# timsainb/noisereduce

Hardware: AMD Instinct MI355X
Metric: Msamples/s reduce_noise (48 kHz mono, n_fft=1024) (higher is better)
Workload: dtype f32

## Files before the change

noisereduce_amd/csrc/fastpath.hpp:

```cpp
#pragma once
#include "kernels.hpp"
#include "thresh.hpp"

namespace sg {

template <int NTHR, int COUNT, typename SLOW>
__device__ __forceinline__ void stage_t2_plain(float* s_t2, const double* __restrict__ T2, int need, double scale, int tid,
                                               SLOW slow) {
  if (need == 0) {
    constexpr int K = (COUNT + NTHR - 1) / NTHR;
    double t[K];
#pragma unroll
    for (int k = 0; k < K; ++k) t[k] = T2[min(tid + k * NTHR, COUNT - 1)];
#pragma unroll
    for (int k = 0; k < K; ++k) {
      const int i = tid + k * NTHR;
      if ((k + 1) * NTHR <= COUNT || i < COUNT) s_t2[i] = t2_to_f32(t[k], scale);
    }
  } else {
    for (int i = tid; i < COUNT; i += NTHR) s_t2[i] = t2_to_f32(slow(i), scale);
  }
}

template <typename ARGS>
__device__ __forceinline__ const ARGS* late_args() {
  const __attribute__((address_space(4))) char* kp = (const __attribute__((address_space(4))) char*)__builtin_amdgcn_kernarg_segment_ptr();
  asm volatile("" : "+s"(kp));
  return reinterpret_cast<const ARGS*>((const char*)kp);
}

namespace fast {

constexpr int FN = 512;
constexpr int FPITCH = FN + 16;
constexpr int WAVE_CX = 4 * FPITCH;
constexpr int FSK = 528;

typedef cx<float> cf;

template <int NTHR, int WIN4>
__device__ __forceinline__ void stage_tables(cf* tw512, const cf* __restrict__ tw_src, float* swin,
                                             const float* __restrict__ win_src, int tid) {
  constexpr bool WIN = WIN4 > 0;
  constexpr int K = (FN + NTHR - 1) / NTHR, KW = WIN ? (WIN4 + NTHR - 1) / NTHR : 1;
  cf t[K];
  float4 w[KW];
#pragma unroll
  for (int k = 0; k < K; ++k) {
    const int i = min(tid + k * NTHR, FN - 1);
    t[k] = tw_src[(i >> 4) * (i & 15)];
  }
  if constexpr (WIN) {
#pragma unroll
    for (int k = 0; k < KW; ++k) w[k] = reinterpret_cast<const float4*>(win_src)[min(tid + k * NTHR, WIN4 - 1)];
  }
#pragma unroll
  for (int k = 0; k < K; ++k) {
    const int i = tid + k * NTHR;
    if ((k + 1) * NTHR <= FN || i < FN) tw512[i] = t[k];
  }
  if constexpr (WIN) {
#pragma unroll
    for (int k = 0; k < KW; ++k) {
      const int i = tid + k * NTHR;
      if ((k + 1) * NTHR <= WIN4 || i < WIN4) reinterpret_cast<float4*>(swin)[i] = w[k];
    }
  }
}
template <int NTHR, int SPAN, int XPITCH, int ROW = 256, bool MX = false>
__device__ __forceinline__ unsigned stage_span_vec(float* xs, const float* __restrict__ sp, int tid) {
  static_assert(SPAN % 4 == 0, "16-byte loads");
  constexpr int N4 = SPAN / 4, NQ = (N4 + NTHR - 1) / NTHR;
  float4 q[NQ];
  unsigned mi = 0u;
#pragma unroll
  for (int k = 0; k < NQ; ++k) q[k] = reinterpret_cast<const float4*>(sp)[min(tid + k * NTHR, N4 - 1)];
#pragma unroll
  for (int k = 0; k < NQ; ++k) {
    const int e = 4 * (tid + k * NTHR);
    if ((k + 1) * NTHR <= N4 || e < SPAN) *reinterpret_cast<float4*>(&xs[(e / ROW) * XPITCH + (e % ROW)]) = q[k];
    if constexpr (MX) {
      auto ab = [](float x) -> unsigned { return __float_as_uint(x) & 0x7fffffffu; };
      mi = max(max(mi, max(ab(q[k].x), ab(q[k].y))), max(ab(q[k].z), ab(q[k].w)));
    }
  }
  return mi;
}

template <int NTHR, int SPAN, int XPITCH, int ROW = 256>
__device__ __forceinline__ void stage_span_vec_i16(float* xs, const int16_t* __restrict__ sp, int tid) {
  static_assert(SPAN % 4 == 0, "8-byte loads");
  constexpr int N4 = SPAN / 4, NQ = (N4 + NTHR - 1) / NTHR;
  uint2 q[NQ];
#pragma unroll
  for (int k = 0; k < NQ; ++k) q[k] = reinterpret_cast<const uint2*>(sp)[min(tid + k * NTHR, N4 - 1)];
#pragma unroll
  for (int k = 0; k < NQ; ++k) {
    const int e = 4 * (tid + k * NTHR);
    const float4 f = {(float)(short)(q[k].x & 0xffffu), (float)((int)q[k].x >> 16), (float)(short)(q[k].y & 0xffffu),
                      (float)((int)q[k].y >> 16)};
    if ((k + 1) * NTHR <= N4 || e < SPAN) *reinterpret_cast<float4*>(&xs[(e / ROW) * XPITCH + (e % ROW)]) = f;
  }
}

__device__ constexpr float C32[9] = {1.0f,
                                     0.98078528040323044913f,
                                     0.92387953251128675613f,
                                     0.83146961230254523708f,
                                     0.70710678118654752440f,
                                     0.55557023301960222474f,
                                     0.38268343236508977173f,
                                     0.19509032201612826785f,
                                     0.0f};

template <int R>
__device__ __forceinline__ constexpr float twc(int k) {
  int j = k * (32 / R);
  return j <= 8 ? C32[j] : -C32[16 - j];
}
template <int R>
__device__ __forceinline__ constexpr float tws(int k) {
  int j = k * (32 / R);
  return j <= 8 ? C32[8 - j] : C32[j - 8];
}

#ifndef SG_PK_FFT
#define SG_PK_FFT 0
#endif
typedef float pf2 __attribute__((ext_vector_type(2)));
__device__ __forceinline__ pf2 pk_of(cf a) { return pf2{a.x, a.y}; }
__device__ __forceinline__ cf pk_to(pf2 a) { return cf{a.x, a.y}; }
__device__ __forceinline__ pf2 pk_add(pf2 a, pf2 b) {
  pf2 d;
  asm("v_pk_add_f32 %0, %1, %2" : "=v"(d) : "v"(a), "v"(b));
  return d;
}
__device__ __forceinline__ pf2 pk_sub(pf2 a, pf2 b) {
  pf2 d;
  asm("v_pk_add_f32 %0, %1, %2 neg_lo:[0,1] neg_hi:[0,1]" : "=v"(d) : "v"(a), "v"(b));
  return d;
}
__device__ __forceinline__ pf2 pk_mul(pf2 a, pf2 b) {
  pf2 d;
  asm("v_pk_mul_f32 %0, %1, %2" : "=v"(d) : "v"(a), "v"(b));
  return d;
}
__device__ __forceinline__ pf2 pk_add_mi(pf2 a, pf2 b) {
  pf2 d;
  asm("v_pk_add_f32 %0, %1, %2 op_sel:[0,1] op_sel_hi:[1,0] neg_hi:[0,1]" : "=v"(d) : "v"(a), "v"(b));
  return d;
}
__device__ __forceinline__ pf2 pk_add_pi(pf2 a, pf2 b) {
  pf2 d;
  asm("v_pk_add_f32 %0, %1, %2 op_sel:[0,1] op_sel_hi:[1,0] neg_lo:[0,1]" : "=v"(d) : "v"(a), "v"(b));
  return d;
// ... 809 lines not shown
        float4 f4 = *reinterpret_cast<const float4*>(&fr[wh * WAVE_CX_H * 2 + lh * HPITCH + s4]);
        acc.x += f4.x; acc.y += f4.y; acc.z += f4.z; acc.w += f4.w;
      }
    } else {
#pragma unroll
      for (int q = 0; q < 4; ++q) {
        const int i = jj - q;
        const int64_t ti = tf_tile + i;
        if (i >= 0 && i < NF && ti >= 0 && ti < G.T) {
          const int off = ((i >> 2) * WAVE_CX + frame_base(i & 3)) * 2 + 256 * q + s4;
          float4 f4 = *reinterpret_cast<const float4*>(&fr[off]);
          acc.x += f4.x; acc.y += f4.y; acc.z += f4.z; acc.w += f4.w;
        }
      }
    }
    if (inkernel && jj >= NF) {
      unsigned long long* dst = A.part2 + (((size_t)u * A.n_tiles + bx) * 3 + (jj - NF)) * 256 + s4;
      const op_v4u ga = {__float_as_uint(acc.x), A.epoch, __float_as_uint(acc.y), A.epoch};
      const op_v4u gb = {__float_as_uint(acc.z), A.epoch, __float_as_uint(acc.w), A.epoch};
      op_st16_sc1(dst, ga);
      op_st16_sc1(dst + 2, gb);
      continue;
    }
    if (inkernel && jj < 3) {
      const unsigned long long* src = A.part2 + (((size_t)u * A.n_tiles + bx - 1) * 3 + jj) * 256 + s4;
      op_v4u ga, gb;
      for (int spin = 0;; ++spin) {
        asm volatile("global_load_dwordx4 %0, %2, off sc1\n\tglobal_load_dwordx4 %1, %2, off offset:16 sc1\n\ts_waitcnt vmcnt(0)"
                     : "=&v"(ga), "=&v"(gb) : "v"(src) : "memory");
        const unsigned e = A.epoch;
        if (!LOSE && ga[1] == e && ga[3] == e && gb[1] == e && gb[3] == e) break;
        if (LOSE || spin >= OP_SPIN_MAX) {
          atomicOr_system(A.err, 4u);
          ga[0] = ga[2] = gb[0] = gb[2] = 0x7fc00000u;
          break;
        }
        __builtin_amdgcn_s_sleep(1);
      }
      acc.x = __uint_as_float(ga[0]) + acc.x;
      acc.y = __uint_as_float(ga[2]) + acc.y;
      acc.z = __uint_as_float(gb[0]) + acc.z;
      acc.w = __uint_as_float(gb[2]) + acc.w;
    } else if (jj < 3 || jj >= NF) {
      const int slot = jj < 3 ? jj : 3 + (jj - NF);
      float* dst = A.part + (((u * A.n_tiles + bx) * 6 + slot) * 256 + s4);
      *reinterpret_cast<float4*>(dst) = acc;
      continue;
    }
    if (!A.normalize) {
    } else if (all_valid) {
      acc.x *= n4.x; acc.y *= n4.y; acc.z *= n4.z; acc.w *= n4.w;
    } else {
      float4 nrm = make_float4(0.f, 0.f, 0.f, 0.f);
#pragma unroll
      for (int q = 0; q < 4; ++q) {
        const int64_t ti = h - q;
        if (ti >= 0 && ti < G.T) {
          float4 w4 = *reinterpret_cast<const float4*>(&A.wsq[256 * q + s4]);
          nrm.x += w4.x; nrm.y += w4.y; nrm.z += w4.z; nrm.w += w4.w;
        }
      }
      acc.x /= (nrm.x > 1e-10f ? nrm.x : 1.f);
      acc.y /= (nrm.y > 1e-10f ? nrm.y : 1.f);
      acc.z /= (nrm.z > 1e-10f ? nrm.z : 1.f);
      acc.w /= (nrm.w > 1e-10f ? nrm.w : 1.f);
    }
    {
      const int64_t pb = h * 256 - G.padL;
      const int64_t gi0 = chunk * A.om.g_step + (pb - A.om.p0);
      if (A.om.dtype == 0 && pb >= A.om.p0 && pb + 256 <= A.om.p1 && pb + 256 <= G.Lout && gi0 >= A.om.g_lo &&
          gi0 + 256 <= A.om.g_hi && !(SG_ABLATE & 4)) {
        float* dst = (float*)A.om.out + (row * A.om.stride + gi0 - A.om.g0 + s4);
        if ((reinterpret_cast<uintptr_t>(dst) & 15) == 0) {
          *reinterpret_cast<float4*>(dst) = acc;
          continue;
        }
      }
    }
    const float vals[4] = {acc.x, acc.y, acc.z, acc.w};
#pragma unroll
    for (int e = 0; e < 4; ++e) {
      const int64_t p = h * 256 + s4 + e - G.padL;
      if (p < A.om.p0 || p >= A.om.p1) continue;
      const int64_t gi = chunk * A.om.g_step + (p - A.om.p0);
      if (gi < A.om.g_lo || gi >= A.om.g_hi) continue;
      if ((SG_ABLATE & 4) && vals[e] != 12345.678f) continue;
      store_sample(A.om.out, A.om.dtype, row * A.om.stride + gi - A.om.g0, p < G.Lout ? vals[e] : 0.f);
    }
  }
}

template <int NF>
__global__ __launch_bounds__(256) void k_ola_seam(ApplyArgs A) {
  const Geom& G = A.g;
  const int64_t u = blockIdx.y;
  const int64_t b = blockIdx.x;
  const int64_t row = (A.view.unit0 + u) / A.view.n_chunks;
  const int64_t chunk = A.view.c0 + (A.view.unit0 + u) % A.view.n_chunks;
  const int s = threadIdx.x;
  const float* pa = A.part + ((u * A.n_tiles + b) * 6 + 3) * 256;
  const float* pb = A.part + ((u * A.n_tiles + b + 1) * 6 + 0) * 256;
#pragma unroll
  for (int k = 0; k < 3; ++k) {
    const int64_t h = A.h_begin - 3 + (int64_t)NF * (b + 1) + k;
    if (h < A.h_begin || h >= A.h_end) continue;
    float val = pa[k * 256 + s] + pb[k * 256 + s];
    if (A.normalize) {
      if (h - 3 >= 0 && h < G.T) {
        val *= A.invn[s];
      } else {
        float nrm = 0.f;
#pragma unroll
        for (int q = 0; q < 4; ++q) {
          const int64_t ti = h - q;
          if (ti >= 0 && ti < G.T) nrm += A.wsq[256 * q + s];
        }
        val /= (nrm > 1e-10f ? nrm : 1.f);
      }
    }
    const int64_t p = h * 256 + s - G.padL;
    if (p < A.om.p0 || p >= A.om.p1) continue;
    const int64_t gi = chunk * A.om.g_step + (p - A.om.p0);
    if (gi < A.om.g_lo || gi >= A.om.g_hi) continue;
    store_sample(A.om.out, A.om.dtype, row * A.om.stride + gi - A.om.g0, p < G.Lout ? val : 0.f);
  }
}

}
}

namespace sg {
namespace fast {

struct DecideArgs {
  View view;
  Geom g;
  const float* win;
  const double* win64;
  const cf* tw512;
  const cf* tw1024;
  const cx<double>* tw64;
  ThreshConsts tc;
  double mag_scale, top_db;
  unsigned long long* bits;
  int wpr;
  int64_t t_begin, t_end;
  int quads_per_wave;
};


__device__ __forceinline__ double exact_power(const DecideArgs& A, int64_t row, int64_t chunk, int64_t t, int f,
                                              int lane) {
  const int64_t s0 = t * A.g.H - A.g.padL;
  double re = 0.0, im = 0.0;
#pragma unroll 4
  for (int i = 0; i < 16; ++i) {
    const int m = lane + 64 * i;
    const double xv = view_sample(A.view, row, chunk, s0 + m) * A.win64[m];
    const int j = (f * m) & 1023;
    cx<double> w = A.tw64[j & 511];
    if (j >= 512) { w.x = -w.x; w.y = -w.y; }
    re += xv * w.x;
    im += xv * w.y;
  }
  for (int off = 32; off > 0; off >>= 1) {
    re += __shfl_xor(re, off);
    im += __shfl_xor(im, off);
  }
  return re * re + im * im;
}

template <int WAVES>
__global__ __launch_bounds__(WAVES * 64, 3) void k_decide_fast(DecideArgs A) {
  extern __shared__ __attribute__((aligned(16))) char smem[];
  cf* tw512 = reinterpret_cast<cf*>(smem);
  cf* regions = tw512 + FN;
  const int tid = threadIdx.x;
  const int lane = tid & 63, wave = tid >> 6;
  const int g = lane >> 4, c = lane & 15;
  const Geom& G = A.g;
  const int64_t u = blockIdx.y;
  const int64_t row = (A.view.unit0 + u) / A.view.n_chunks;
  const int64_t chunk = A.view.c0 + (A.view.unit0 + u) % A.view.n_chunks;
  const int need = A.tc.need_floor[u];
  const bool floor_live = need == 1;

  float* s_t2 = reinterpret_cast<float*>(regions + WAVES * WAVE_CX_H);
  auto t2eff = [&](int f) -> double {
    double v = A.tc.T2[f];
    if (floor_live) {
      double fl = cell_db(A.tc.pmax[u * G.FS + f], A.mag_scale) - A.top_db;
      if (fl > A.tc.thresh[f]) v = -1.0;
    }
    if (need == 2) v = T2_NEVER;
    return v;
  };
  for (int i = tid; i <= 512; i += WAVES * 64) {
    double v = t2eff(perm_inv(i));
    s_t2[t2_pos(i)] = t2_to_f32(v, 4.0);
  }
  cf* fb = regions + wave * WAVE_CX_H + frame_base_h(g);
  const cf wl0 = A.tw1024[c];
  float* swin = s_t2 + T2_FLOATS;
  stage_tables<WAVES * 64, 256>(tw512, A.tw512, swin, A.win, tid);
  constexpr int NFB = 4 * WAVES, SPAN = (NFB - 1) * 256 + 1024, XPITCH = 288;
  static_assert((SPAN / 256) * XPITCH <= WAVES * WAVE_CX_H * 2, "span must fit the exchange slices");
  const int64_t tqb = A.t_begin + (int64_t)blockIdx.x * NFB;
  bool blk_vec;
  {
    const int64_t s0b = tqb * 256 - G.padL;
    const int64_t gb = chunk * A.view.cs - A.view.pad + s0b;
    const float* sp = (const float*)A.view.x + row * A.view.stride + gb;
    const bool interior = tqb + NFB <= A.t_end && tqb + NFB <= G.T && s0b >= 0 && s0b + SPAN <= A.view.Lp &&
                          gb >= A.view.lo && gb + SPAN <= A.view.hi;
    const int16_t* sp16 = (const int16_t*)A.view.x + row * A.view.stride + gb;
    const bool vec16 = A.view.dtype == 2 && interior && (reinterpret_cast<uintptr_t>(sp16) & 7) == 0;
    blk_vec = (A.view.dtype == 0 && interior && (reinterpret_cast<uintptr_t>(sp) & 15) == 0) || vec16;
    float* xs = reinterpret_cast<float*>(regions);
    if (vec16) {
      stage_span_vec_i16<WAVES * 64, SPAN, XPITCH>(xs, sp16, tid);
    } else if (blk_vec) {
      stage_span_vec<WAVES * 64, SPAN, XPITCH>(xs, sp, tid);
    } else {
      for (int i = tid; i < SPAN; i += WAVES * 64)
        xs[(i >> 8) * XPITCH + (i & 255)] = (float)view_sample(A.view, row, chunk, s0b + i);
    }
  }
  __syncthreads();

  {
    const int64_t tq = tqb + wave * 4;
    const int64_t t = tq + g;
    const bool fvalid = t < A.t_end && t < G.T;
    cf v[32];
    float nrm2 = 0.f;
    {
      const float* xs = reinterpret_cast<const float*>(regions) + (4 * wave + g) * XPITCH + 2 * c;
      const float2* wl2 = reinterpret_cast<const float2*>(swin + 2 * c);
      if (blk_vec) {
#pragma unroll
        for (int r = 0; r < 32; ++r) {
          const float2 x2 = *reinterpret_cast<const float2*>(xs + (r >> 3) * XPITCH + 32 * (r & 7));
          const float2 w2 = wl2[16 * r];
          v[r] = {x2.x * w2.x, x2.y * w2.y};
        }
      } else {
#pragma unroll
        for (int r = 0; r < 32; ++r) {
          float2 x2 = *reinterpret_cast<const float2*>(xs + (r >> 3) * XPITCH + 32 * (r & 7));
          if (!fvalid) x2 = make_float2(0.f, 0.f);
          const float2 w2 = wl2[16 * r];
          v[r] = {x2.x * w2.x, x2.y * w2.y};
        }
      }
    }
    __syncthreads();
    if (tq >= A.t_end) return;
    {
#pragma unroll
      for (int r = 0; r < 32; ++r) nrm2 += v[r].x * v[r].x + v[r].y * v[r].y;
      nrm2 += __shfl_xor(nrm2, 1);
      nrm2 += __shfl_xor(nrm2, 2);
      nrm2 += __shfl_xor(nrm2, 4);
      nrm2 += __shfl_xor(nrm2, 8);
    }
    {
      int z0 = 0;
      asm volatile("" : "+v"(z0));
      fft512_fwd_half(v, fb, tw512 + z0, c);
    }
    cf wl = wl0;
    asm volatile("" : "+v"(wl.x), "+v"(wl.y));
    float t2[32];
    float t2_512;
    {
      int zt = 0;
      asm volatile("" : "+v"(zt));
      const float* tp = s_t2 + zt;
      const float4* t4 = reinterpret_cast<const float4*>(tp + c * T2_PITCH);
#pragma unroll
      for (int q4 = 0; q4 < 8; ++q4) {
        float4 x = t4[q4];
        t2[4 * q4] = x.x; t2[4 * q4 + 1] = x.y; t2[4 * q4 + 2] = x.z; t2[4 * q4 + 3] = x.w;
      }
      t2_512 = tp[T2_POS512];
    }

    const float d2 = nrm2 > 0.f ? 8.0f * 2.3283064e-10f * nrm2 : -1.0f;
    unsigned pred = 0, amb = 0;
    auto decide = [&](float P, float T, int q) {
      const float diff = P - T;
      pred |= (diff > 0.f ? 1u : 0u) << q;
      amb |= ((diff * diff <= d2 * (P + T)) ? 1u : 0u) << q;
    };
    auto pair_power = [&](cf a, cf b, cf w, float& Pk, float& Pn) {
      cf p, q;
      split_pair(a, b, w, p, q);
      Pk = p.x * p.x + p.y * p.y;
      Pn = q.x * q.x + q.y * q.y;
    };
    const bool l0 = c == 0;
    const cf wlo = wl;
    cf whi = wl;
    {
      const cf w16 = A.tw1024[16];
      if (l0) whi = {-w16.y, w16.x};
    }
    auto sel = [&](cf a0, cf a1) -> cf { return {l0 ? a0.x : a1.x, l0 ? a0.y : a1.y}; };
    bool pred512 = false, amb512 = false;
    {
      float Pk, Pn;
      pair_power(v[0], v[31], wlo, Pk, Pn);
      const cf a = v[0];
      const float x0 = 2.f * (a.x + a.y), xN = 2.f * (a.x - a.y);
      const float P256 = 4.f * (v[8].x * v[8].x + v[8].y * v[8].y);
      decide(l0 ? x0 * x0 : Pk, t2[0], 0);
      decide(l0 ? P256 : Pn, t2[31], 31);
      const float P5 = xN * xN, d5 = P5 - t2_512;
      pred512 = l0 && d5 > 0.f;
      amb512 = l0 && d5 * d5 <= d2 * (P5 + t2_512);
    }
#pragma unroll
// ... 239 lines not shown
```

noisereduce_amd/csrc/onepass.hpp:

```cpp
#pragma once
#include "fastpath.hpp"

namespace sg {
namespace fast {

constexpr int OP_XW = 9;
constexpr int OP_TILE_WORDS = 16 * OP_XW * 2;
constexpr int OP_MAX_NT = 16;
constexpr int OP_KP = 528;
constexpr int OP_TAB_WIN = 0, OP_TAB_WSQ = 4096, OP_TAB_INVN = 8192, OP_TAB_TW512 = 9216, OP_TAB_TW1024 = 13312,
              OP_TAB_WIN64 = 17408, OP_TAB_TW64 = 25600, OP_TAB_MCONST = 33792, OP_TAB_EXP8 = 35328, OP_TAB_BYTES = 37376;

#ifndef OP_LATE_ARGS
#define OP_LATE_ARGS 1
#endif
#ifndef OP_TRACE
#define OP_TRACE 0
#endif
#ifndef OP_ARGCHECK
#define OP_ARGCHECK 0
#endif
#ifndef OP_TILECOUNT
#define OP_TILECOUNT 0
#endif
#ifndef OP_NO_LOOPTOP_WAIT
#define OP_NO_LOOPTOP_WAIT 0
#endif
#ifndef OP_BACKOFF
#define OP_BACKOFF 0
#endif
#if OP_BACKOFF
#define OP_POLL_SLEEP(spin) do { if ((spin) >= 8) __builtin_amdgcn_s_sleep(127); else __builtin_amdgcn_s_sleep(1); } while (0)
#else
#define OP_POLL_SLEEP(spin) __builtin_amdgcn_s_sleep(1)
#endif
#ifndef OP_WHO
#define OP_WHO 0
#endif
#ifndef OP_GLOBAL_DRAW
#define OP_GLOBAL_DRAW 0
#endif
#if OP_GLOBAL_DRAW
#define OP_DRAW_TICKET(p64) __hip_atomic_fetch_add((__attribute__((address_space(1))) unsigned*)(p64), 1u, __ATOMIC_RELAXED, __HIP_MEMORY_SCOPE_AGENT)
#else
#define OP_DRAW_TICKET(p64) atomicAdd((unsigned*)(uintptr_t)(p64), 1u)
#endif
#ifndef OP_DRAW_TOP
#define OP_DRAW_TOP 0
#endif
#ifndef OP_RESTAGE
#define OP_RESTAGE 0
#endif
#ifndef OP_MAX_ITERS
#define OP_MAX_ITERS 0
#endif
#ifndef OP_LATE_START_US
#define OP_LATE_START_US 0
#endif
#ifndef OP_EXP_STALL_NS
#define OP_EXP_STALL_NS 0
#endif
#ifndef OP_INPLACE
#define OP_INPLACE 0
#endif
struct OnePassArgs {
  ApplyArgs A;
  const void* x_exact;
  int64_t stride_exact;
  int dtype_exact;
  const char* tab;
  ThreshConsts tc;
  double mag_scale, top_db;
  unsigned long long* xbits;
  unsigned* ticket;
  unsigned ticket_base;
  unsigned epoch;
  unsigned* err;
  int nf, nt;
  float prop, inv_ktot;
  unsigned long long* part2;
  unsigned* alim;
  int scan_q;
  unsigned total_tiles;
#if OP_TRACE
  unsigned* trace;
#endif
#if OP_WHO
  unsigned* who;
#endif
};

#if OP_LATE_ARGS
#define OP_XARG(type, member) (*(const __attribute__((address_space(4))) type*)(kp4 + __builtin_offsetof(OnePassArgs, member)))
#else
#define OP_XARG(type, member) (P.member)
#endif
__device__ __forceinline__ double op_exact_power(const OnePassArgs& P, int64_t row, int64_t chunk, int64_t t, int f,
                                                 int lane) {
#if OP_LATE_ARGS
  const __attribute__((address_space(4))) char* kp4 = (const __attribute__((address_space(4))) char*)__builtin_amdgcn_kernarg_segment_ptr();
  asm volatile("" : "+s"(kp4));
#endif
  const int64_t s0 = t * OP_XARG(int32_t, A.g.H) - OP_XARG(int32_t, A.g.padL);
  const int64_t v_cs = OP_XARG(int64_t, A.view.cs), v_pad = OP_XARG(int64_t, A.view.pad), v_Lp = OP_XARG(int64_t, A.view.Lp),
                v_lo = OP_XARG(int64_t, A.view.lo), v_hi = OP_XARG(int64_t, A.view.hi), x_stride = OP_XARG(int64_t, stride_exact);
  const void* const x_exact = (const void*)(uintptr_t)OP_XARG(unsigned long long, x_exact);
  const int x_dtype = OP_XARG(int, dtype_exact);
  const char* const tab = (const char*)(uintptr_t)OP_XARG(unsigned long long, tab);
  double re = 0.0, im = 0.0;
#pragma unroll 4
  for (int i = 0; i < 16; ++i) {
    const int m = lane + 64 * i;
    double xs = 0.0;
    {
      const int64_t sp = s0 + m;
      const int64_t gi = chunk * v_cs - v_pad + sp;
      if (sp >= 0 && sp < v_Lp && gi >= v_lo && gi < v_hi) xs = load_sample(x_exact, x_dtype, row * x_stride + gi);
    }
    const double xv = xs * reinterpret_cast<const double*>(tab + OP_TAB_WIN64)[m];
    const int j = (f * m) & 1023;
    cx<double> w = reinterpret_cast<const cx<double>*>(tab + OP_TAB_TW64)[j & 511];
    if (j >= 512) { w.x = -w.x; w.y = -w.y; }
    re += xv * w.x;
    im += xv * w.y;
  }
  for (int off = 32; off > 0; off >>= 1) {
    re += __shfl_xor(re, off);
    im += __shfl_xor(im, off);
  }
  return re * re + im * im;
}

__device__ __forceinline__ unsigned op_nan_bits() {
  unsigned v = 0x7fc00000u;
  asm volatile("" : "+v"(v));
  return v;
}

#ifndef OP_ABLATE
#define OP_ABLATE 0
#endif
#ifndef OP_TRACE
#define OP_TRACE 0
#endif
#if OP_TRACE
#define OP_STAMP(i)                                                                                   \
  do {                                                                                                \
    const long long t_now_ = clock64();                                                               \
    if (lane == 0 && t_slot_) t_slot_[i] = (unsigned)(t_now_ - t_prev_);                              \
    t_prev_ = t_now_;                                                                                 \
  } while (0)
#else
#define OP_STAMP(i) do { } while (0)
#endif

#ifndef OP_LATE_P
#define OP_LATE_P 1
#endif
#ifndef OP_OCC
#define OP_OCC 3
#endif
#define OP_DONE { if (PERSIST) continue; return; }
#ifndef OP_DEFER_SEAM
#define OP_DEFER_SEAM 1
#endif
constexpr unsigned OP_SEAM_NONE = 0xffffffffu;
template <int WAVES, bool PROP, bool LOSE = false, bool REDO = false, bool PERSIST = false>
__global__ __launch_bounds__(WAVES * 64, OP_OCC) void k_gate_onepass(OnePassArgs Pk) {
  static_assert(WAVES == 4, "tile = 16 frames");
  static_assert(!PERSIST || (!LOSE && !REDO), "the persistent loop is the lazy first launch only");
  extern __shared__ __attribute__((aligned(16))) char smem[];
  cf* tw512 = reinterpret_cast<cf*>(smem);
  cf* regions = tw512 + FN;
  float* swin = reinterpret_cast<float*>(regions + WAVES * WAVE_CX_H);
  float* s_t2 = swin + 1024;
  unsigned long long* s_exp = reinterpret_cast<unsigned long long*>(s_t2 + T2_FLOATS);
  double* s_t2d = reinterpret_cast<double*>(s_exp + 256);
  unsigned* s_misc = reinterpret_cast<unsigned*>(s_t2d + 514);
  unsigned char* s_ef = reinterpret_cast<unsigned char*>(s_misc + 8);
  constexpr int NF = 4 * WAVES;
  constexpr int SPAN = (NF - 1) * 256 + 1024, XPITCH = 288;
  static_assert((SPAN / 256) * XPITCH <= WAVES * WAVE_CX_H * 2, "span must fit the exchange slices");
  constexpr int NQ = SPAN / 256;
  static_assert(SPAN % 256 == 0 && WAVES * 64 == 256, "one sample per thread and row");
  constexpr int SCAN_REG = 5;

  if (REDO && Pk.alim[1] != Pk.tc.need_tag) return;
#if OP_LATE_START_US
  if (PERSIST && (blockIdx.x % 5u) == 1u) {
    const unsigned long long t0_ = wall_clock64();
    while ((long long)(wall_clock64() - t0_) < (long long)OP_LATE_START_US * 100 * (1 + (blockIdx.x % 7u))) __builtin_amdgcn_s_sleep(8);
  }
#endif
  double t2pre[3];
  unsigned alim_v = 0u;
  {
    const int tid = threadIdx.x, lane = tid & 63;
    static_assert(FN == 2 * WAVES * 64 && WAVES * 64 == 256, "one pass of the prologue loads per thread");
    const cf tw_a = reinterpret_cast<const cf*>(Pk.tab + OP_TAB_TW512)[(tid >> 4) * (tid & 15)];
    const cf tw_b = reinterpret_cast<const cf*>(Pk.tab + OP_TAB_TW512)[((tid + 256) >> 4) * (tid & 15)];
    const float4 w4 = reinterpret_cast<const float4*>(Pk.tab + OP_TAB_WIN)[tid];
    const unsigned long long e8 = reinterpret_cast<const unsigned long long*>(Pk.tab + OP_TAB_EXP8)[tid];
    t2pre[0] = Pk.tc.T2[perm_inv(tid)];
    t2pre[1] = Pk.tc.T2[perm_inv(tid + 256)];
    t2pre[2] = Pk.tc.T2[perm_inv(512)];
    if (!REDO && Pk.alim != nullptr) {
      int z = 2 + min(lane & 15, OP_ALIM_BLOCKS - 1);
      asm volatile("" : "+v"(z));
      alim_v = Pk.alim[z];
    }
    if (tid == 0) {
      s_misc[PERSIST ? 4 : 0] = Pk.ticket_base == 0xffffffffu ? blockIdx.x : atomicAdd(Pk.ticket, 1u) - Pk.ticket_base;
      s_misc[1] = 0u;
      if (PERSIST) s_misc[0] = OP_SEAM_NONE;
    }
    tw512[tid] = tw_a;
    tw512[tid + 256] = tw_b;
    reinterpret_cast<float4*>(swin)[tid] = w4;
    s_exp[tid] = e8;
    if constexpr (PROP) {
      for (int f = tid; f <= 512; f += WAVES * 64) {
        const int lo = max(-Pk.nf, -f), hi = min(Pk.nf, 512 - f);
        int sum = 0;
        for (int a = lo; a <= hi; ++a) sum += Pk.nf + 1 - (a < 0 ? -a : a);
        s_ef[f] = (unsigned char)sum;
      }
    }
    if constexpr (PERSIST) {
#pragma unroll
      for (int k = 0; k < 3; ++k) {
        const int i = tid + k * WAVES * 64;
        if (i > 512) break;
        s_t2[t2_pos(i)] = t2_to_f32(t2pre[k], 4.0);
        s_t2d[i] = t2pre[k];
      }
      for (int off = 1; off < 16; off <<= 1) alim_v = min(alim_v, (unsigned)__shfl_xor((int)alim_v, off));
      if (tid == 0) s_misc[2] = alim_v;
#if OP_TILECOUNT == 2
      if (tid == 0) { s_misc[3] = Pk.total_tiles; s_misc[6] = (unsigned)(uintptr_t)Pk.err; s_misc[7] = (unsigned)((uintptr_t)Pk.err >> 32); }
#endif
    }
  }
  __syncthreads();

  struct TileSrc {
    const float* sp;
    bool blk_vec;
    const float* sc_base;
    int sc_n1;
    int64_t s0b, sc_lo, sc_last, sc_lenA, sc_c0, sc_c1;
  };
  auto tile_src = [](const OnePassArgs& P, int64_t row, int64_t chunk, int jt, bool test) -> TileSrc {
    const ApplyArgs& A = P.A;
    TileSrc S;
    const int64_t tf_tile = A.h_begin - 3 + (int64_t)jt * NF;
    S.s0b = tf_tile * 256 - A.g.padL;
    const int64_t gb = chunk * A.view.cs - A.view.pad + S.s0b;
    S.sp = (const float*)A.view.x + row * A.view.stride + gb;
    S.blk_vec = A.view.dtype == 0 && tf_tile >= 0 && tf_tile + NF <= A.g.T && S.s0b >= 0 && S.s0b + SPAN <= A.view.Lp &&
                gb >= A.view.lo && gb + SPAN <= A.view.hi && (reinterpret_cast<uintptr_t>(S.sp) & 15) == 0;
    S.sc_base = nullptr;
    S.sc_n1 = 0;
    S.sc_lo = S.sc_last = S.sc_lenA = S.sc_c0 = S.sc_c1 = 0;
    if (test) {
      const int64_t g0 = chunk * A.view.cs - A.view.pad;
      const int64_t s_lo = max<int64_t>(0, A.view.lo - g0), s_hi = min<int64_t>(A.view.Lp, A.view.hi - g0);
      const int64_t sp0 = (A.h_begin - 3 - NF) * 256 - A.g.padL;
      const int64_t sp1 = (A.h_begin - 3 + (int64_t)A.n_tiles * NF) * 256 - A.g.padL + SPAN;
      const int64_t first = min(s_hi, max(s_lo, sp0));
      S.sc_lo = s_lo;
      S.sc_last = max(s_lo, min(s_hi, sp1));
      S.sc_lenA = first - s_lo;
      S.sc_c0 = (int64_t)(jt + 1) * P.scan_q;
      S.sc_c1 = min(S.sc_c0 + P.scan_q, S.sc_lenA + (s_hi - S.sc_last));
      if (A.view.dtype == 0 && S.sc_c1 > S.sc_c0 && S.sc_c1 - S.sc_c0 <= SCAN_REG * WAVES * 64 &&
          (S.sc_c1 <= S.sc_lenA || S.sc_c0 >= S.sc_lenA)) {
        S.sc_base = (const float*)A.view.x + row * A.view.stride + g0 +
                    (S.sc_c1 <= S.sc_lenA ? s_lo + S.sc_c0 : S.sc_last + (S.sc_c0 - S.sc_lenA));
        S.sc_n1 = (int)(S.sc_c1 - S.sc_c0) - 1;
      }
    }
    return S;
  };
// ... 1039 lines not shown
```

Before: 103,300.

## Rewrite exact single-bin DFT power with Horner recurrence and cross-lane reduction

Replaces the per-sample twiddle-table lookup in the exact fp64 single-bin DFT power check with a Horner-style recurrence. Each lane multiplies by a uniform rotation factor, so only one per-lane twiddle is loaded at the end. It precomputes valid sample bounds once instead of doing per-sample bounds checks, and uses uniform scalar pointers. The final reduction uses permlane32_swap plus ds_swizzle instead of shfl_xor. This exact-recheck path only runs for borderline threshold decisions, and the Horner form changes fp64 rounding order slightly.

Result: faster. 105,000 (median of 6 runs) (+1.7%).

```diff
diff --git a/noisereduce_amd/csrc/exact1024.hpp b/noisereduce_amd/csrc/exact1024.hpp
--- /dev/null
+++ b/noisereduce_amd/csrc/exact1024.hpp
@@ -0,0 +1,108 @@
+#pragma once
+#include "fft_wave.hpp"
+#include "geom.hpp"
+
+namespace sg {
+namespace fast {
+
+__device__ __forceinline__ void exact1024_terms(int64_t s0, int64_t e, int64_t Lp, int64_t lo, int64_t hi, int& a, int& b) {
+  const int64_t first = -s0 > lo - e ? -s0 : lo - e;
+  const int64_t end = Lp - s0 < hi - e ? Lp - s0 : hi - e;
+  a = (int)(first < 0 ? 0 : first > 1024 ? 1024 : first);
+  b = (int)(end < 0 ? 0 : end > 1024 ? 1024 : end);
+}
+
+__device__ __forceinline__ double ex_uniform(double v) {
+  return __hiloint2double(__builtin_amdgcn_readfirstlane(__double2hiint(v)), __builtin_amdgcn_readfirstlane(__double2loint(v)));
+}
+
+template <typename T>
+using ex_gptr = const __attribute__((address_space(1))) T*;
+template <typename T>
+__device__ __forceinline__ ex_gptr<T> ex_global(const T* p) {
+  const unsigned long long v = (unsigned long long)(uintptr_t)p;
+  const unsigned lo = (unsigned)__builtin_amdgcn_readfirstlane((int)(unsigned)v), hi = (unsigned)__builtin_amdgcn_readfirstlane((int)(unsigned)(v >> 32));
+  return (ex_gptr<T>)(uintptr_t)((unsigned long long)lo | ((unsigned long long)hi << 32));
+}
+
+template <int OFF>
+__device__ __forceinline__ double ex_swz_xor(double v) {
+  constexpr int pat = (OFF << 10) | 0x1f;
+  return __hiloint2double(__builtin_amdgcn_ds_swizzle(__double2hiint(v), pat), __builtin_amdgcn_ds_swizzle(__double2loint(v), pat));
+}
+
+template <typename T, int I0>
+__device__ __forceinline__ void ex_horner8(ex_gptr<T> xa, ex_gptr<double> win64, int lane, int la, int n, double rx, double ry,
+                                           double& hr, double& hi) {
+  T xs[8];
+  double wv[8];
+#pragma unroll
+  for (int i = 0; i < 8; ++i) {
+    const int r = la + 64 * (I0 + i);
+    const int rc = r < 0 ? 0 : r >= n ? n - 1 : r;
+    xs[i] = *(ex_gptr<T>)((ex_gptr<char>)xa + (unsigned)rc * (unsigned)sizeof(T));
+    wv[i] = *(ex_gptr<double>)((ex_gptr<char>)win64 + (unsigned)(lane + 64 * (I0 + i)) * 8u);
+  }
+  __builtin_amdgcn_sched_barrier(0);
+  asm volatile("" : "+v"(la));
+#pragma unroll
+  for (int i = 7; i >= 0; --i) {
+    const int r = la + 64 * (I0 + i);
+    const double xv = ((unsigned)r < (unsigned)n ? (double)xs[i] : 0.0) * wv[i];
+    const double nr = fma(hr, rx, fma(-hi, ry, xv));
+    hi = fma(hr, ry, hi * rx);
+    hr = nr;
+  }
+}
+
+template <typename T>
+__device__ __forceinline__ double ex_power_t(const T* xp, int a, int b, const double* win64_, const cx<double>* tw64_,
+                                             int f, int lane) {
+  asm volatile("" : "+v"(lane));
+  const ex_gptr<T> xa = ex_global(xp + a);
+  const ex_gptr<double> win64 = ex_global(win64_);
+  const ex_gptr<double> tw64 = ex_global(reinterpret_cast<const double*>(tw64_));
+  const int n = b - a, la = lane - a;
+  const int jl = (f * lane) & 1023, jr = (f * 64) & 1023;
+  const ex_gptr<double> pl = (ex_gptr<double>)((ex_gptr<char>)tw64 + (unsigned)(jl & 511) * 16u);
+  const ex_gptr<double> pr = (ex_gptr<double>)((ex_gptr<char>)tw64 + (unsigned)(jr & 511) * 16u);
+  cx<double> wl = {pl[0], pl[1]}, rho = {pr[0], pr[1]};
+  double h0r, h0i, h1r, h1i;
+  {
+    if (jr >= 512) { rho.x = -rho.x; rho.y = -rho.y; }
+    const double rx = ex_uniform(rho.x), ry = ex_uniform(rho.y);
+    h0r = h0i = h1r = h1i = 0.0;
+    ex_horner8<T, 0>(xa, win64, lane, la, n, rx, ry, h0r, h0i);
+    ex_horner8<T, 8>(xa, win64, lane, la, n, rx, ry, h1r, h1i);
+  }
+  if (jl >= 512) { wl.x = -wl.x; wl.y = -wl.y; }
+  const double sr = (f & 1) ? h0r - h1r : h0r + h1r, si = (f & 1) ? h0i - h1i : h0i + h1i;
+  const double re = fma(sr, wl.x, -(si * wl.y)), im = fma(sr, wl.y, si * wl.x);
+  const auto s_lo = __builtin_amdgcn_permlane32_swap((unsigned)__double2loint(re), (unsigned)__double2loint(im), false, false);
+  const auto s_hi = __builtin_amdgcn_permlane32_swap((unsigned)__double2hiint(re), (unsigned)__double2hiint(im), false, false);
+  double v = __hiloint2double((int)s_hi[0], (int)s_lo[0]) + __hiloint2double((int)s_hi[1], (int)s_lo[1]);
+  v += ex_swz_xor<16>(v);
+  v += ex_swz_xor<8>(v);
+  v += ex_swz_xor<4>(v);
+  v += ex_swz_xor<2>(v);
+  v += ex_swz_xor<1>(v);
+  const int v_lo = __double2loint(v), v_hi = __double2hiint(v);
+  const double tr = __hiloint2double(__builtin_amdgcn_readlane(v_hi, 0), __builtin_amdgcn_readlane(v_lo, 0));
+  const double ti = __hiloint2double(__builtin_amdgcn_readlane(v_hi, 32), __builtin_amdgcn_readlane(v_lo, 32));
+  return fma(tr, tr, ti * ti);
+}
+
+__device__ __forceinline__ double exact1024_power(const void* x, int dtype, int64_t e0, int a, int b, const double* win64,
+                                                  const cx<double>* tw64, int f, int lane) {
+  if (a >= b) return 0.0;
+  f = __builtin_amdgcn_readfirstlane(f);
+  switch (dtype) {
+    case 0: return ex_power_t((const float*)x + e0, a, b, win64, tw64, f, lane);
+    case 1: return ex_power_t((const double*)x + e0, a, b, win64, tw64, f, lane);
+    case 2: return ex_power_t((const int16_t*)x + e0, a, b, win64, tw64, f, lane);
+    default: return ex_power_t((const int32_t*)x + e0, a, b, win64, tw64, f, lane);
+  }
+}
+
+}
+}
diff --git a/noisereduce_amd/csrc/fastpath.hpp b/noisereduce_amd/csrc/fastpath.hpp
--- a/noisereduce_amd/csrc/fastpath.hpp
+++ b/noisereduce_amd/csrc/fastpath.hpp
@@ -1,6 +1,7 @@
 #pragma once
 #include "kernels.hpp"
 #include "thresh.hpp"
+#include "exact1024.hpp"
 
 namespace sg {
 
@@ -1116,22 +1117,10 @@
 __device__ __forceinline__ double exact_power(const DecideArgs& A, int64_t row, int64_t chunk, int64_t t, int f,
                                               int lane) {
   const int64_t s0 = t * A.g.H - A.g.padL;
-  double re = 0.0, im = 0.0;
-#pragma unroll 4
-  for (int i = 0; i < 16; ++i) {
-    const int m = lane + 64 * i;
-    const double xv = view_sample(A.view, row, chunk, s0 + m) * A.win64[m];
-    const int j = (f * m) & 1023;
-    cx<double> w = A.tw64[j & 511];
-    if (j >= 512) { w.x = -w.x; w.y = -w.y; }
-    re += xv * w.x;
-    im += xv * w.y;
-  }
-  for (int off = 32; off > 0; off >>= 1) {
-    re += __shfl_xor(re, off);
-    im += __shfl_xor(im, off);
-  }
-  return re * re + im * im;
+  const int64_t e = chunk * A.view.cs - A.view.pad + s0;
+  int a, b;
+  exact1024_terms(s0, e, A.view.Lp, A.view.lo, A.view.hi, a, b);
+  return exact1024_power(A.view.x, A.view.dtype, row * A.view.stride + e, a, b, A.win64, A.tw64, f, lane);
 }
 
 template <int WAVES>
diff --git a/noisereduce_amd/csrc/onepass.hpp b/noisereduce_amd/csrc/onepass.hpp
--- a/noisereduce_amd/csrc/onepass.hpp
+++ b/noisereduce_amd/csrc/onepass.hpp
@@ -107,28 +107,11 @@
   const void* const x_exact = (const void*)(uintptr_t)OP_XARG(unsigned long long, x_exact);
   const int x_dtype = OP_XARG(int, dtype_exact);
   const char* const tab = (const char*)(uintptr_t)OP_XARG(unsigned long long, tab);
-  double re = 0.0, im = 0.0;
-#pragma unroll 4
-  for (int i = 0; i < 16; ++i) {
-    const int m = lane + 64 * i;
-    double xs = 0.0;
-    {
-      const int64_t sp = s0 + m;
-      const int64_t gi = chunk * v_cs - v_pad + sp;
-      if (sp >= 0 && sp < v_Lp && gi >= v_lo && gi < v_hi) xs = load_sample(x_exact, x_dtype, row * x_stride + gi);
-    }
-    const double xv = xs * reinterpret_cast<const double*>(tab + OP_TAB_WIN64)[m];
-    const int j = (f * m) & 1023;
-    cx<double> w = reinterpret_cast<const cx<double>*>(tab + OP_TAB_TW64)[j & 511];
-    if (j >= 512) { w.x = -w.x; w.y = -w.y; }
-    re += xv * w.x;
-    im += xv * w.y;
-  }
-  for (int off = 32; off > 0; off >>= 1) {
-    re += __shfl_xor(re, off);
-    im += __shfl_xor(im, off);
-  }
-  return re * re + im * im;
+  const int64_t e = chunk * v_cs - v_pad + s0;
+  int a, b;
+  exact1024_terms(s0, e, v_Lp, v_lo, v_hi, a, b);
+  return exact1024_power(x_exact, x_dtype, row * x_stride + e, a, b, reinterpret_cast<const double*>(tab + OP_TAB_WIN64),
+                         reinterpret_cast<const cx<double>*>(tab + OP_TAB_TW64), f, lane);
 }
 
 __device__ __forceinline__ unsigned op_nan_bits() {
```
